# CAMMA-public/SelfPose3d

Hardware: AMD Instinct MI355X
Metric: multi-view samples/sec (5-view Panoptic, 80x80x20 voxel) (higher is better)
Workload: dtype f32

## Files before the change

include/sp3d.h:

```cpp
#ifndef SP3D_H
#define SP3D_H

#include <stdint.h>

#ifdef __cplusplus
extern "C" {
#endif

#define SP3D_ABI_VERSION 3
#define SP3D_MAX_VIEWS 16
#define SP3D_MAX_TOPK 32

#define SP3D_CAM_STRIDE 64
#define SP3D_CAM_R 0
#define SP3D_CAM_T 9
#define SP3D_CAM_F 12
#define SP3D_CAM_C 14
#define SP3D_CAM_K 16
#define SP3D_CAM_P 19
#define SP3D_CAM_A 21
#define SP3D_CAM_W0 27
#define SP3D_CAM_H0 28
#define SP3D_CAM_FLIP 29
#define SP3D_CAM_RXY 32
// ... 147 lines not shown
int sp3d_wino_fused_split(const float *x, const void *U3, float *y, const float *shift, const float *residual, int mode, int B,
                          int X, int Y, int Z, int C, int O, void *stream);

int sp3d_wino_fused_split64(const float *x, const void *U3, float *y, const float *shift, const float *residual, int mode,
                            int B, int X, int Y, int Z, int C, int O, void *stream);

int sp3d_conv3_split(const float *x, const void *W3, float *y, const float *shift, const float *residual, int mode, int B,
                     int X, int Y, int Z, int C, int O, void *stream);

int sp3d_upsample2x_scatter(const float *G, float *out, const float *shift, const float *skip, int64_t batch, int X, int Y,
                            int Z, int O, void *stream);

int sp3d_upsample2x_scatter_head(const float *G, float *head, const float *shift, const float *skip, const float *wout,
                                 const float *bout, int64_t batch, int X, int Y, int Z, int O, int J, void *stream);

#define SP3D_GBN_F32 0
#define SP3D_GBN_F64 1
#define SP3D_GBN_REPLICAS 16
#define SP3D_GBN_PLAIN 0
#define SP3D_GBN_RELU 1
#define SP3D_GBN_ADD_RELU 2
int64_t sp3d_gbn_workspace_bytes(int G, int C);
int sp3d_gbn_forward(const void *x, void *y, int dtype, const int32_t *group_of, const int32_t *group_samples, int N,
                     int64_t S, int C, int G, int G_update, const void *weight, const void *bias, void *running_mean,
                     void *running_var, double eps, double momentum, int mode, const void *residual, void *mean,
                     void *invstd, void *scale, void *shift, double *workspace, void *stream);
int sp3d_gbn_backward(const void *x, const void *dy, void *dx, int dtype, const int32_t *group_of,
                      const int32_t *group_samples, int N, int64_t S, int C, int G, const void *weight, const void *mean,
                      const void *invstd, const void *scale, const void *shift, int mode, const void *y,
                      void *grad_residual, void *grad_weight, void *grad_bias, void *k123, double *workspace, void *stream);
// ... 6 lines not shown
```

selfpose3d_amd/_lib.py:

```python
from __future__ import annotations

import ctypes as C
import os
from typing import Optional, Sequence

import torch

_HERE = os.path.dirname(os.path.abspath(__file__))
_DEFAULT_LIB_PATH = os.path.join(_HERE, "libsp3d.so")
NOPK_LIB_PATH = os.path.join(_HERE, "libsp3d_nopk.so")
LIB_PATH = os.environ.get("SP3D_LIB_PATH") or _DEFAULT_LIB_PATH

LAYOUT_PLANAR = 0
LAYOUT_NHWC = 1
OUT_CHANNELS_LAST = 0x100
HM_BF16 = 0x200
OUT_BF16 = 0x400
SCATTER_AUTO, SCATTER_PER_TAP, SCATTER_MERGE = 0, 2, 3
MAX_VIEWS = 16
MAX_TOPK = 32
ABI_VERSION = 3

EXPORTS = [
    "sp3d_abi_version", "sp3d_error_string", "sp3d_pack_heatmaps", "sp3d_unproject_fwd", "sp3d_unproject_bwd",
    "sp3d_nms_topk_workspace_bytes", "sp3d_nms_topk", "sp3d_nms_proposals", "sp3d_soft_argmax", "sp3d_unproject_fwd_indexed",
    "sp3d_unproject_bwd_indexed", "sp3d_unproject_fwd_strided", "sp3d_fetch_ring", "sp3d_maxpool2x_cl", "sp3d_crop_shift_act_cl", "sp3d_rfft3d", "sp3d_irfft3d", "sp3d_cfft2d", "sp3d_cfft2d_ex", "sp3d_zdft_fwd_cl", "sp3d_zdft_inv_cl", "sp3d_unproject_fwd_zdft", "sp3d_cfft2d_88_tiled", "sp3d_freq_contract_ty", "sp3d_soft_argmax_grid", "sp3d_soft_argmax_grid_train", "sp3d_soft_argmax_grid_bwd", "sp3d_channel_shift_act", "sp3d_pack_heatmaps_ex",
    "sp3d_unproject_fwd_train", "sp3d_unproject_bwd_packed", "sp3d_unproject_bwd_packed_det", "sp3d_fixed_to_float", "sp3d_gaussian_target_3d", "sp3d_render_root_heatmaps", "sp3d_freq_contract", "sp3d_freq_contract_ex", "sp3d_wino_input", "sp3d_wino_output", "sp3d_wino_fused", "sp3d_wino_fused_split", "sp3d_wino_fused_split64", "sp3d_conv3_split", "sp3d_camera_finish", "sp3d_upsample2x_scatter", "sp3d_upsample2x_scatter_head", "sp3d_render_joints_fwd", "sp3d_render_joints_bwd", "sp3d_gbn_workspace_bytes", "sp3d_gbn_forward", "sp3d_gbn_backward",
]

_lib = None


class Sp3dError(RuntimeError):
    pass


def shared_gpu() -> bool:
    v = os.environ.get("SP3D_SHARED_GPU")
    if v is not None:
        return v.lower() in ("1", "true", "yes", "on")
    if any(os.environ.get(k) not in (None, "") for k in ("HIP_VISIBLE_DEVICES", "CUDA_VISIBLE_DEVICES", "ROCR_VISIBLE_DEVICES",
                                                          "GPU_DEVICE_ORDINAL")):
# ... 749 lines not shown
    if not x.is_contiguous(memory_format=torch.channels_last_3d) or x.dtype != torch.float32:
        raise Sp3dError("upsample2x_head_: float32 channels_last_3d activations expected")
    O = int(w_gemm.shape[1]) // 8
    J = int(w_out.shape[0])
    G = torch.matmul(x.permute(0, 2, 3, 4, 1).reshape(-1, Cc), w_gemm)
    if tuple(skip.shape) != (B, O, 2 * X, 2 * Y, 2 * Z) or not skip.is_contiguous(memory_format=torch.channels_last_3d):
        skip = skip.contiguous(memory_format=torch.channels_last_3d)
    wo = w_out.reshape(J, O).contiguous().float()
    bo = (b_out if b_out is not None else torch.zeros(J, device=x.device)).contiguous().float()
    head = torch.empty((B, 2 * X, 2 * Y, 2 * Z, J), dtype=torch.float32, device=x.device)
    check(lib.sp3d_upsample2x_scatter_head(G.data_ptr(), head.data_ptr(), shift.data_ptr(), skip.data_ptr(), wo.data_ptr(),
                                           bo.data_ptr(), B, X, Y, Z, O, J, _stream(x.device)), "sp3d_upsample2x_scatter_head")
    return head.permute(0, 4, 1, 2, 3)


class _RenderJoints(torch.autograd.Function):
    @staticmethod
    def forward(ctx, kps, count, h, w, sigma):
        lib = load()
        _require_cuda(kps, "kps")
        N, Pn, J = (int(v) for v in kps.shape[:3])
        k = kps.contiguous().float()
        cnt = None if count is None else count.to(device=kps.device, dtype=torch.int32).contiguous()
        out = torch.empty((N, J, h, w), dtype=torch.float32, device=kps.device)
        check(lib.sp3d_render_joints_fwd(k.data_ptr(), cnt.data_ptr() if cnt is not None else None, N, Pn, J, h, w,
                                         float(sigma), out.data_ptr(), _stream(kps.device)), "sp3d_render_joints_fwd")
        ctx.save_for_backward(k, cnt if cnt is not None else torch.empty(0, device=kps.device))
        ctx.geom = (h, w, float(sigma), cnt is not None, kps.dtype)
        return out if kps.dtype == torch.float32 else out.to(kps.dtype)

# ... 16 lines not shown
```

selfpose3d_amd/build.py:

```python
from __future__ import annotations

import os
import subprocess
import sys

HERE = os.path.dirname(os.path.abspath(__file__))
CSRC = os.path.join(HERE, "csrc")
SOURCES = ["sp3d_unproject.hip", "sp3d_proposal.hip", "sp3d_epilogue.hip", "sp3d_synth.hip", "sp3d_fftconv.hip", "sp3d_winograd.hip", "sp3d_fft.hip", "sp3d_gbn.hip"]
HEADERS = [os.path.join("..", "pk_src1.py"), "sp3d_device.h", "sp3d_proj_pk.h", "sp3d_tuning.h", "sp3d_twiddles.h", os.path.join("..", "..", "include", "sp3d.h")]
LIB = os.path.join(HERE, "libsp3d.so")
HIPCC = os.environ.get("HIPCC", "/opt/rocm/bin/hipcc")
FLAGS = ["--offload-arch=gfx950", "-O3", "-std=c++17", "-ffp-contract=off", "-munsafe-fp-atomics", "-fPIC", "-shared",
         "-Wall", "-Wno-unused-function"]
LINK = ["-L/opt/rocm/lib", "-lhipfft"]


def needs_build() -> bool:
    if not os.path.exists(LIB):
        return True
    t = os.path.getmtime(LIB)
    deps = [os.path.join(CSRC, s) for s in SOURCES + HEADERS] + [os.path.abspath(__file__)]
    return any(os.path.getmtime(d) > t for d in deps if os.path.exists(d))


PER_SOURCE_FLAGS = {"sp3d_winograd.hip": ["-fno-slp-vectorize"],
                    "sp3d_fft.hip": ["-fno-slp-vectorize"], "sp3d_fftconv.hip": ["-fno-slp-vectorize"]}


LLVM_BIN = os.environ.get("SP3D_LLVM_BIN", "/opt/rocm/lib/llvm/bin")

NOPK_LIB = os.path.join(HERE, "libsp3d_nopk.so")
NOPK_FLAGS = ["-DSP3D_NO_PK", "-fno-slp-vectorize", "-Xclang", "-target-feature", "-Xclang", "-packed-fp32-ops"]




def _compile_one(src: str, objdir: str, cflags, verbose: bool, host_flags=()) -> str:
    from . import pk_src1
    base = os.path.join(objdir, src.replace(".hip", ""))
    path = os.path.join(CSRC, src)
    cuid = "-cuid=" + src.replace(".", "_")
# ... 85 lines not shown
```

selfpose3d_amd/csrc/sp3d_winograd.hip:

```cpp
#include <hip/hip_runtime.h>
#include <stdint.h>

#include "../../include/sp3d.h"

namespace sp3d {

__device__ __forceinline__ void bt4(float &d0, float &d1, float &d2, float &d3)
{
    const float t0 = d0 - d2, t1 = d1 + d2, t2 = d2 - d1, t3 = d1 - d3;
    d0 = t0; d1 = t1; d2 = t2; d3 = t3;
}

__global__ __launch_bounds__(256) void wino_input_kernel(const float *__restrict__ x, float *__restrict__ V, int B, int X,
                                                        int Y, int Z, int C, int TX, int TY, int TZ)
{
    const int64_t T = (int64_t)B * TX * TY * TZ;
    const int64_t gid = (int64_t)blockIdx.x * 256 + threadIdx.x;
    if (gid >= T * C) return;
    const int c = (int)(gid % C);
    int64_t t = gid / C;
    const int tz = (int)(t % TZ); int64_t r = t / TZ;
    const int ty = (int)(r % TY); r /= TY;
    const int tx = (int)(r % TX);
    const int b = (int)(r / TX);
// ... 858 lines not shown

__device__ __forceinline__ void split3(const float4 a, u32x4 &q0, u32x4 &q1)
{
    const unsigned hi01 = pack_bf16(a.x, a.y), hi23 = pack_bf16(a.z, a.w);
    const float r0 = __builtin_amdgcn_fmed3f(a.x - bf16_lo(hi01), 0.0f, a.x - bf16_lo(hi01));
    const float r1 = __builtin_amdgcn_fmed3f(a.y - bf16_hi(hi01), 0.0f, a.y - bf16_hi(hi01));
    const float r2 = __builtin_amdgcn_fmed3f(a.z - bf16_lo(hi23), 0.0f, a.z - bf16_lo(hi23));
    const float r3 = __builtin_amdgcn_fmed3f(a.w - bf16_hi(hi23), 0.0f, a.w - bf16_hi(hi23));
    const unsigned mid01 = pack_bf16(r0, r1), mid23 = pack_bf16(r2, r3);
    const unsigned lo01 = pack_bf16(r0 - bf16_lo(mid01), r1 - bf16_hi(mid01));
    const unsigned lo23 = pack_bf16(r2 - bf16_lo(mid23), r3 - bf16_hi(mid23));
    q0 = u32x4{lo01, lo23, hi01, hi23};
    q1 = u32x4{hi01, hi23, mid01, mid23};
}

template <int C, int MODE>
__global__ __launch_bounds__(64 * (4 + CD_PROD)) __attribute__((amdgpu_waves_per_eu(2, 2)))
void conv3_split_kernel(const float *__restrict__ x, const unsigned *__restrict__ W3, float *__restrict__ y,
                        const float *__restrict__ shift, const float *__restrict__ res, int B, int X, int Y, int Z, int NBX,
                        int NBY, int NBZ, int nblocks)
{
    constexpr int O = 32, NCH = C / 8;
    extern __shared__ __attribute__((aligned(16))) unsigned cd_lds[];
    const int tid = threadIdx.x, lane = tid & 63, wave = tid >> 6, t = lane & 31, h = lane >> 5;
    const int my_blocks = ((int)blockIdx.x < nblocks) ? (nblocks - 1 - (int)blockIdx.x) / (int)gridDim.x + 1 : 0;
    const int n_items = my_blocks * NCH;
    auto decode = [&](int item, int &b, int &ox0, int &oy0, int &oz0) {
        int bid = (int)blockIdx.x + (item / NCH) * (int)gridDim.x;
        const int bz = bid % NBZ; bid /= NBZ;
        const int by = bid % NBY; bid /= NBY;
        const int bx = bid % NBX;
        b = bid / NBX;
        ox0 = bx * CD_BX; oy0 = by * CD_BY; oz0 = bz * CD_BZ;
    };

// ... 121 lines not shown
            }
#pragma unroll
            for (int r = 0; r < 9; ++r) {
                __builtin_amdgcn_sched_group_barrier(0x008, 1, 0);
                __builtin_amdgcn_sched_group_barrier(0x020, 1, 0);
            }
            __builtin_amdgcn_sched_group_barrier(0x008, 15, 0);
            __builtin_amdgcn_sched_barrier(0);
            a0 = a1;
            w0 = w1;
        }
        CD_STAMP(1);
        if (cc == NCH - 1) {
            int b, ox0, oy0, oz0;
            decode(item, b, ox0, oy0, oz0);
            if (ox0 + CD_BX <= X && oy0 + CD_BY <= Y && oz0 + CD_BZ <= Z) {
                const float sh = shift[t];
                const int64_t obase = ((((int64_t)b * X + ox0 + 4 * wave) * Y + oy0 + 4 * h) * Z + oz0) * O + t;
#pragma unroll
                for (int i = 0; i < 4; ++i)
#pragma unroll
                    for (int v = 0; v < 16; ++v) {
                        const int64_t idx = obase + (((int64_t)i * Y + (v & 3)) * Z + (v >> 2)) * O;
                        float val = acc[i][v] + sh;
                        if (MODE == 2) val += res[idx];
                        if (MODE >= 1) val = fmaxf(val, 0.0f);
                        if (MODE == 3) val += res[idx];
#if SP3D_W16_ABLATE & 16
                        if (val == 123.456f)
#endif
                        y[idx] = val;
// ... 9 lines not shown
                __builtin_amdgcn_fence(__ATOMIC_RELEASE, "wavefront");
                __builtin_amdgcn_wave_barrier();
#pragma unroll
                for (int r = 0; r < 4; ++r) {
                    const int m = (lane >> 3) + 8 * r;
                    float4 a = *reinterpret_cast<const float4 *>(scr + m * 32 + 4 * g);
                    const int xo = ox0 + 4 * wave + mb, yo = oy0 + (m & 7), zo = oz0 + (m >> 3);
                    if (xo < X && yo < Y && zo < Z) {
                        const int64_t vox = (((int64_t)b * X + xo) * Y + yo) * Z + zo;
                        a.x += sh4.x; a.y += sh4.y; a.z += sh4.z; a.w += sh4.w;
                        float4 rr = make_float4(0.0f, 0.0f, 0.0f, 0.0f);
                        if (MODE >= 2) rr = *reinterpret_cast<const float4 *>(res + vox * O + 4 * g);
                        if (MODE == 2) { a.x += rr.x; a.y += rr.y; a.z += rr.z; a.w += rr.w; }
                        if (MODE >= 1) { a.x = fmaxf(a.x, 0.0f); a.y = fmaxf(a.y, 0.0f); a.z = fmaxf(a.z, 0.0f); a.w = fmaxf(a.w, 0.0f); }
                        if (MODE == 3) { a.x += rr.x; a.y += rr.y; a.z += rr.z; a.w += rr.w; }
#if SP3D_W16_ABLATE & 16
                        if (a.x == 123.456f)
#endif
                        *reinterpret_cast<float4 *>(y + vox * O + 4 * g) = a;
                    }
                }
                __builtin_amdgcn_fence(__ATOMIC_RELEASE, "wavefront");
                __builtin_amdgcn_wave_barrier();
            }
            }
        }
        CD_STAMP(2);
        __syncthreads();
        CD_STAMP(3);
    }
}


}
// ... 63 lines not shown
    const int64_t blocks = (int64_t)B * NBX * NBY * NBZ;
    if (blocks > 0x7fffffff) return SP3D_ERANGE;
    constexpr int nbw = 2, ks = 2;
    hipStream_t s = (hipStream_t)stream;
    const unsigned *u3 = reinterpret_cast<const unsigned *>(U3);
    const dim3 grid((unsigned)blocks), block(64 * (4 / nbw) * ks);
#define SP3D_WF(C_, M_) hipLaunchKernelGGL((wino_fused16_kernel<C_, M_, 2, 2>), grid, block, 0, s, x, u3, y, shift, residual, B, X, Y, Z, NBX, NBY, NBZ)
#define SP3D_WFM(C_) switch (mode) { case 0: SP3D_WF(C_, 0); break; case 1: SP3D_WF(C_, 1); break; case 2: SP3D_WF(C_, 2); break; default: SP3D_WF(C_, 3); }
    if (C == 32) { SP3D_WFM(32) } else { SP3D_WFM(64) }
#undef SP3D_WFM
#undef SP3D_WF
    const hipError_t e = hipGetLastError();
    return e == hipSuccess ? SP3D_OK : (int)e;
}

extern "C" int sp3d_conv3_split(const float *x, const void *W3, float *y, const float *shift, const float *residual, int mode,
                                int B, int X, int Y, int Z, int C, int O, void *stream)
{
    using namespace sp3d;
    if (B <= 0 || X <= 0 || Y <= 0 || Z <= 0 || mode < 0 || mode > 3) return SP3D_EINVAL;
    if (!x || !W3 || !y || !shift || (mode >= 2 && !residual)) return SP3D_ENULL;
    if (O != 32 || (C != 16 && C != 32) || (reinterpret_cast<uintptr_t>(W3) & 15)) return SP3D_EUNSUPPORTED;
    if (reinterpret_cast<uintptr_t>(y) & 15) return SP3D_EUNSUPPORTED;
    if ((int64_t)X * Y * Z * C * 2 > 0x7fffffff) return SP3D_ERANGE;
    const int NBX = (X + CD_BX - 1) / CD_BX, NBY = (Y + CD_BY - 1) / CD_BY, NBZ = (Z + CD_BZ - 1) / CD_BZ;
    const int64_t blocks = (int64_t)B * NBX * NBY * NBZ;
    if (blocks > 0x7fffffff) return SP3D_ERANGE;
    static int cu_count[64] = {0};
    int dev = 0, cus = 256;
    if (hipGetDevice(&dev) == hipSuccess && dev >= 0 && dev < 64) {
        if (cu_count[dev] == 0) {
            int n = 0;
            cu_count[dev] = (hipDeviceGetAttribute(&n, hipDeviceAttributeMultiprocessorCount, dev) == hipSuccess && n > 0) ? n : 256;
        }
        cus = cu_count[dev];
    }
    const int rounds = (int)((blocks + cus - 1) / cus);
    const int nwg = (int)((blocks + rounds - 1) / rounds);
    const dim3 grid((unsigned)nwg), block(64 * (4 + CD_PROD));
    const size_t lds = (size_t)2 * CD_BUFS * sizeof(unsigned) + 4 * 1024 * sizeof(float);
    hipStream_t s = (hipStream_t)stream;
    const unsigned *w3 = reinterpret_cast<const unsigned *>(W3);
    int cd_dev = 0;
    { const hipError_t ed = hipGetDevice(&cd_dev); if (ed != hipSuccess) return (int)ed; }
    if (cd_dev < 0 || cd_dev >= 64) cd_dev = 63;
#define SP3D_CD(C_, M_) { static bool attr_dev[64] = {}; bool &attr = attr_dev[cd_dev]; if (!attr || cd_dev == 63) { hipError_t ea = hipFuncSetAttribute(reinterpret_cast<const void *>(conv3_split_kernel<C_, M_>), hipFuncAttributeMaxDynamicSharedMemorySize, (int)lds); if (ea != hipSuccess) return (int)ea; attr = true; } \
    hipLaunchKernelGGL((conv3_split_kernel<C_, M_>), grid, block, lds, s, x, w3, y, shift, residual, B, X, Y, Z, NBX, NBY, NBZ, (int)blocks); }
#define SP3D_CDI(C_) switch (mode) { case 0: SP3D_CD(C_, 0); break; case 1: SP3D_CD(C_, 1); break; case 2: SP3D_CD(C_, 2); break; default: SP3D_CD(C_, 3); }
    if (C == 16) { SP3D_CDI(16) } else { SP3D_CDI(32) }
#undef SP3D_CDI
#undef SP3D_CD
    const hipError_t e = hipGetLastError();
    return e == hipSuccess ? SP3D_OK : (int)e;
}

extern "C" int sp3d_debug_conv3_timeline(void *dev_buffer)
{
#ifdef SP3D_CD_TIMELINE
    unsigned long long *p = (unsigned long long *)dev_buffer;
    return (int)hipMemcpyToSymbol(HIP_SYMBOL(sp3d::g_cd_tl), &p, sizeof(p));
#else
    (void)dev_buffer;
    return SP3D_EUNSUPPORTED;
#endif
}
```

selfpose3d_amd/v2v_net.py:

```python
from __future__ import annotations

import torch
import torch.nn as nn
import torch.nn.functional as F


def _bn(c):
    from .grouped_bn import GroupedBatchNorm3d
    return GroupedBatchNorm3d(c)


def _grouped(bn, training: bool) -> bool:
    return training and getattr(bn, "groups", None) is not None


def fft_len(n: int) -> int:
    m = n + (n & 1)
    while True:
        r, odd = m, 0
        for q in (2, 3, 5, 7, 11, 13):
            if q > 2 and r % q == 0:
                odd += 1
            while r % q == 0:
                r //= q
# ... 185 lines not shown
                    u._sp3d_direct = _lib.conv_weights_split(wc)
            for u in (u1, u2):
                if u is not None and u.shape[2] == 32 and u.shape[1] in (16, 32):
                    u._sp3d_split = _lib.wino_weights_split(u)
                elif u is not None and u.shape[2] == 64 and u.shape[1] in (32, 64):
                    u._sp3d_split = _lib.wino_weights_split(u, 16)
            if len(blk.skip_con) > 0:
                ws, ss = self._fold(blk.skip_con[0], blk.skip_con[1])
                t[name] = (w1, s1, w2, (s2 + ss).contiguous(), ws, u1, u2)
            else:
                t[name] = (w1, s1, w2, s2, None, u1, u2)
        res("front_res", n.front_layers[1])
        ed = n.encoder_decoder
        for name in ("encoder_res1", "encoder_res2", "mid_res", "decoder_res2", "decoder_res1", "skip_res1", "skip_res2"):
            res(name, getattr(ed, name))
        for name in ("decoder_upsample2", "decoder_upsample1"):
            blk = getattr(ed, name).block
            wT, sT = self._fold(blk[0], blk[1], transposed=True)
            wg = wT.permute(0, 2, 3, 4, 1).reshape(wT.shape[0], 8 * wT.shape[1]).contiguous()
            t[name] = (wT, sT, wg)
        self.t = t

    def _conv3(self, x, w, u, shift, mode, residual=None):
        from . import _lib
        if u is not None and self.net.winograd and x.is_contiguous(memory_format=torch.channels_last_3d) \
                and not x.is_contiguous():
            B, C, X, Y, Z = x.shape
            T = B * ((X + 1) // 2) * ((Y + 1) // 2) * ((Z + 1) // 2)
            u3 = getattr(u, "_sp3d_split", None) if getattr(self.net, "wino_split", True) else None
            if u3 is not None and u.shape[2] == 64:
                return _lib.wino_fused_conv3d_(x, u, shift, mode, residual, u3)
            if C >= 128 or (C >= 64 and 64 * T * C * 4 <= 160e6):
                return _lib.wino_conv3d_(x, u, shift, mode, residual)
            w3 = getattr(u, "_sp3d_direct", None) if getattr(self.net, "wino_split", True) and getattr(self.net, "direct_conv", True) else None
# ... 203 lines not shown
        else:
            buf = self._fft_buffer(B, cin, S, x.device)
            buf[:, :, :X, :Y, :Z].copy_(x[:, :cin])
        Yf = _lib.freq_contract(_lib.rfft3d(buf), self.t[wkey])
        y = _lib.irfft3d_(Yf, S[2])
        w1 = self.t["front_res"][0]
        cl = w1.is_contiguous(memory_format=torch.channels_last_3d) and not w1.is_contiguous()
        if cl and y.is_contiguous() and y.shape[1] % 4 == 0 and Z % 4 == 0 and 4 * Z * (y.shape[1] + 4) * 4 <= 65536:
            return _lib.crop_shift_act_cl(y, X, Y, Z, s0, True)
        y = y[:, :, :X, :Y, :Z]
        y = y.contiguous(memory_format=torch.channels_last_3d if cl else torch.contiguous_format)
        return _lib.channel_shift_act_(y, s0, 1)

    def _tail(self, x):
        from . import _lib
        x = self._res(x, "front_res")
        skip1 = self._res(x, "skip_res1")
        x = self._res(self._pool(x), "encoder_res1")
        skip2 = self._res(x, "skip_res2")
        x = self._res(self._pool(x), "encoder_res2")
        x = self._res(self._res(x, "mid_res"), "decoder_res2")
        x = self._up2x(x, "decoder_upsample2", skip2)
        x = self._res(x, "decoder_res1")
        o = self.net.output_layer
        wT, sT, wg = self.t["decoder_upsample1"]
        if self.net.winograd and self._is_cl(x) and wg.is_cuda and wT.shape[1] == 32 and x.dtype == torch.float32:
            return _lib.upsample2x_head_(x, wg, sT, skip1, o.weight, o.bias)
        x = self._up2x(x, "decoder_upsample1", skip1)
        return self._conv1(x, o.weight, o.bias)

    def _pool(self, x):
        from . import _lib
        if self._is_cl(x) and x.is_cuda and x.dtype == torch.float32 and x.shape[1] % 4 == 0 and \
                all(int(v) % 2 == 0 for v in x.shape[2:]):
            return _lib.maxpool2x(x)
        return F.max_pool3d(x, 2, 2)

    @staticmethod
    def _is_cl(x):
        return x.is_contiguous(memory_format=torch.channels_last_3d) and not x.is_contiguous()

    def _up2x(self, x, name, skip):
        from . import _lib
        wT, sT, wg = self.t[name]
        if self.net.winograd and self._is_cl(x) and wg.is_cuda and wT.shape[1] % 4 == 0:
            return _lib.upsample2x_(x, wg, sT, skip)
        return _lib.channel_shift_act_(F.conv_transpose3d(x, wT, None, 2), sT, 3, skip)

    def _conv1(self, x, w, bias=None):
        if self.net.winograd and self._is_cl(x) and x.is_cuda:
            B, C, X, Y, Z = x.shape
            O = w.shape[0]
            x2 = x.permute(0, 2, 3, 4, 1).reshape(-1, C)
            y = torch.matmul(x2, w.reshape(O, C).t()) if bias is None else torch.addmm(bias, x2, w.reshape(O, C).t())
            return y.view(B, X, Y, Z, O).permute(0, 4, 1, 2, 3)
        return F.conv3d(x, w, bias, 1, 0)


class V2VNet(nn.Module):
    def __init__(self, input_channels: int, output_channels: int):
        super().__init__()
        self.front_layers = nn.Sequential(ConvBnRelu3d(input_channels, 16, 7), Residual3d(16, 32))
# ... 97 lines not shown
```

Measured before the change: 2746.

## Fuse transposed-conv upsample GEMM with scatter and output head via split-bf16 MFMA

Adds a new kernel that does the 2x transposed-conv upsample as an in-kernel GEMM on bf16 MFMA units. It splits operands into hi/mid/lo bf16 pieces to keep near-f32 accuracy, and fuses the shift, skip add and scatter into the same kernel. This replaces the torch.matmul intermediate G plus a separate scatter kernel. A head variant also folds the final 1x1 output conv into the epilogue. An optional path fuses the J-channel head into the skip_res1 conv3 kernel, off by default. The aim is to cut the intermediate tensor's memory traffic and launches, at the cost of extra MFMA work for the precision split and heavy LDS use.

```diff
diff --git a/include/sp3d.h b/include/sp3d.h
--- a/include/sp3d.h
+++ b/include/sp3d.h
@@ -185,6 +185,16 @@
 int sp3d_upsample2x_scatter_head(const float *G, float *head, const float *shift, const float *skip, const float *wout,
                                  const float *bout, int64_t batch, int X, int Y, int Z, int O, int J, void *stream);
 
+int sp3d_upsample2x_gemm(const float *x, const void *W3, float *out, const float *shift, const float *skip, int B, int X,
+                         int Y, int Z, int C, int O, void *stream);
+
+int sp3d_upsample2x_gemm_head(const float *x, const void *W3, float *head, const float *shift, const float *skip,
+                              const float *wout, const float *bout, int B, int X, int Y, int Z, int C, int O, int J,
+                              int skip_j, void *stream);
+
+int sp3d_conv3_split_head(const float *x, const void *W3, float *head, const float *shift, const float *residual,
+                          const float *wout, int B, int X, int Y, int Z, int C, int O, int J, void *stream);
+
 #define SP3D_GBN_F32 0
 #define SP3D_GBN_F64 1
 #define SP3D_GBN_REPLICAS 16
diff --git a/selfpose3d_amd/_lib.py b/selfpose3d_amd/_lib.py
--- a/selfpose3d_amd/_lib.py
+++ b/selfpose3d_amd/_lib.py
@@ -25,7 +25,7 @@
     "sp3d_abi_version", "sp3d_error_string", "sp3d_pack_heatmaps", "sp3d_unproject_fwd", "sp3d_unproject_bwd",
     "sp3d_nms_topk_workspace_bytes", "sp3d_nms_topk", "sp3d_nms_proposals", "sp3d_soft_argmax", "sp3d_unproject_fwd_indexed",
     "sp3d_unproject_bwd_indexed", "sp3d_unproject_fwd_strided", "sp3d_fetch_ring", "sp3d_maxpool2x_cl", "sp3d_crop_shift_act_cl", "sp3d_rfft3d", "sp3d_irfft3d", "sp3d_cfft2d", "sp3d_cfft2d_ex", "sp3d_zdft_fwd_cl", "sp3d_zdft_inv_cl", "sp3d_unproject_fwd_zdft", "sp3d_cfft2d_88_tiled", "sp3d_freq_contract_ty", "sp3d_soft_argmax_grid", "sp3d_soft_argmax_grid_train", "sp3d_soft_argmax_grid_bwd", "sp3d_channel_shift_act", "sp3d_pack_heatmaps_ex",
-    "sp3d_unproject_fwd_train", "sp3d_unproject_bwd_packed", "sp3d_unproject_bwd_packed_det", "sp3d_fixed_to_float", "sp3d_gaussian_target_3d", "sp3d_render_root_heatmaps", "sp3d_freq_contract", "sp3d_freq_contract_ex", "sp3d_wino_input", "sp3d_wino_output", "sp3d_wino_fused", "sp3d_wino_fused_split", "sp3d_wino_fused_split64", "sp3d_conv3_split", "sp3d_camera_finish", "sp3d_upsample2x_scatter", "sp3d_upsample2x_scatter_head", "sp3d_render_joints_fwd", "sp3d_render_joints_bwd", "sp3d_gbn_workspace_bytes", "sp3d_gbn_forward", "sp3d_gbn_backward",
+    "sp3d_unproject_fwd_train", "sp3d_unproject_bwd_packed", "sp3d_unproject_bwd_packed_det", "sp3d_fixed_to_float", "sp3d_gaussian_target_3d", "sp3d_render_root_heatmaps", "sp3d_freq_contract", "sp3d_freq_contract_ex", "sp3d_wino_input", "sp3d_wino_output", "sp3d_wino_fused", "sp3d_wino_fused_split", "sp3d_wino_fused_split64", "sp3d_conv3_split", "sp3d_camera_finish", "sp3d_upsample2x_scatter", "sp3d_upsample2x_scatter_head", "sp3d_upsample2x_gemm", "sp3d_upsample2x_gemm_head", "sp3d_conv3_split_head", "sp3d_render_joints_fwd", "sp3d_render_joints_bwd", "sp3d_gbn_workspace_bytes", "sp3d_gbn_forward", "sp3d_gbn_backward",
 ]
 
 _lib = None
@@ -805,6 +805,97 @@
     return head.permute(0, 4, 1, 2, 3)
 
 
+def upsample_weights_split(w_gemm: torch.Tensor) -> torch.Tensor:
+    Cc, N = (int(v) for v in w_gemm.shape)
+    w = w_gemm.float()
+    hi = w.bfloat16()
+    r = w - hi.float()
+    mid = r.bfloat16()
+    lo = (r - mid.float()).bfloat16()
+    pieces = torch.stack([lo, hi, mid, hi], 0).reshape(4, Cc // 8, 2, 4, N)
+    return pieces.permute(1, 2, 4, 0, 3).contiguous()
+
+
+def _upsample_args(x: torch.Tensor, W3: torch.Tensor, shift: torch.Tensor, skip: torch.Tensor, skip_c: Optional[int],
+                   what: str):
+    _require_cuda(x, "x")
+    B, Cc, X, Y, Z = (int(v) for v in x.shape)
+    if not x.is_contiguous(memory_format=torch.channels_last_3d) or x.dtype != torch.float32:
+        raise Sp3dError(f"{what}: float32 channels_last_3d activations expected")
+    if W3.dtype != torch.bfloat16 or not W3.is_contiguous() or tuple(W3.shape[:2]) != (Cc // 8, 2) or W3.shape[2] % 8:
+        raise Sp3dError(f"{what}: weight records of upsample_weights_split expected")
+    O = int(W3.shape[2]) // 8
+    if shift.dtype != torch.float32 or not shift.is_contiguous() or shift.numel() != O or shift.device != x.device:
+        raise Sp3dError(f"{what}: shift must be {O} contiguous float32 values on the activations' device")
+    want = (B, O if skip_c is None else skip_c, 2 * X, 2 * Y, 2 * Z)
+    if skip.dtype != torch.float32 or tuple(skip.shape) != want or skip.device != x.device:
+        raise Sp3dError(f"{what}: float32 skip of shape {want} expected")
+    if not skip.is_contiguous(memory_format=torch.channels_last_3d):
+        skip = skip.contiguous(memory_format=torch.channels_last_3d)
+    return B, Cc, X, Y, Z, O, skip
+
+
+def upsample2x_gemm_(x: torch.Tensor, W3: torch.Tensor, shift: torch.Tensor, skip: torch.Tensor) -> torch.Tensor:
+    lib = load()
+    B, Cc, X, Y, Z, O, skip = _upsample_args(x, W3, shift, skip, None, "upsample2x_gemm_")
+    out = torch.empty((B, 2 * X, 2 * Y, 2 * Z, O), dtype=torch.float32, device=x.device).permute(0, 4, 1, 2, 3)
+    lib.sp3d_upsample2x_gemm.restype = C.c_int
+    lib.sp3d_upsample2x_gemm.argtypes = [C.c_void_p] * 5 + [C.c_int] * 6 + [C.c_void_p]
+    check(lib.sp3d_upsample2x_gemm(x.data_ptr(), W3.data_ptr(), out.data_ptr(), shift.data_ptr(), skip.data_ptr(), B, X, Y,
+                                   Z, Cc, O, _stream(x.device)), "sp3d_upsample2x_gemm")
+    return out
+
+
+def _head_weights(w_out: torch.Tensor, b_out: Optional[torch.Tensor], O: int, device):
+    J = int(w_out.shape[0])
+    if w_out.numel() != J * O:
+        raise Sp3dError(f"head weights: (J, {O}, 1, 1, 1) expected, got {tuple(w_out.shape)}")
+    wo = w_out.reshape(J, O).contiguous().float()
+    bo = (b_out if b_out is not None else torch.zeros(J, device=device)).contiguous().float()
+    if bo.numel() != J:
+        raise Sp3dError(f"head bias: {J} values expected")
+    return J, wo, bo
+
+
+def upsample2x_gemm_head_(x: torch.Tensor, W3: torch.Tensor, shift: torch.Tensor, skip: torch.Tensor, w_out: torch.Tensor,
+                          b_out: torch.Tensor, skip_head: bool = False) -> torch.Tensor:
+    lib = load()
+    J = int(w_out.shape[0])
+    B, Cc, X, Y, Z, O, skip = _upsample_args(x, W3, shift, skip, J if skip_head else None, "upsample2x_gemm_head_")
+    J, wo, bo = _head_weights(w_out, b_out, O, x.device)
+    head = torch.empty((B, 2 * X, 2 * Y, 2 * Z, J), dtype=torch.float32, device=x.device)
+    lib.sp3d_upsample2x_gemm_head.restype = C.c_int
+    lib.sp3d_upsample2x_gemm_head.argtypes = [C.c_void_p] * 7 + [C.c_int] * 8 + [C.c_void_p]
+    check(lib.sp3d_upsample2x_gemm_head(x.data_ptr(), W3.data_ptr(), head.data_ptr(), shift.data_ptr(), skip.data_ptr(),
+                                        wo.data_ptr(), bo.data_ptr(), B, X, Y, Z, Cc, O, J, int(bool(skip_head)),
+                                        _stream(x.device)), "sp3d_upsample2x_gemm_head")
+    return head.permute(0, 4, 1, 2, 3)
+
+
+def conv3_split_head_(x: torch.Tensor, W3: torch.Tensor, shift: torch.Tensor, residual: torch.Tensor,
+                      w_out: torch.Tensor) -> torch.Tensor:
+    lib = load()
+    _require_cuda(x, "x")
+    B, Cc, X, Y, Z = (int(v) for v in x.shape)
+    if not x.is_contiguous(memory_format=torch.channels_last_3d) or x.dtype != torch.float32:
+        raise Sp3dError("conv3_split_head_: float32 channels_last_3d activations expected")
+    O = int(W3.shape[3])
+    J = int(w_out.shape[0])
+    if w_out.numel() != J * O:
+        raise Sp3dError(f"head weights: (J, {O}, 1, 1, 1) expected, got {tuple(w_out.shape)}")
+    wo = w_out.reshape(J, O).contiguous().float()
+    if tuple(residual.shape) != (B, O, X, Y, Z) or residual.dtype != torch.float32:
+        raise Sp3dError("conv3_split_head_: float32 residual of the result's shape expected")
+    if not residual.is_contiguous(memory_format=torch.channels_last_3d):
+        residual = residual.contiguous(memory_format=torch.channels_last_3d)
+    head = torch.empty((B, X, Y, Z, J), dtype=torch.float32, device=x.device)
+    lib.sp3d_conv3_split_head.restype = C.c_int
+    lib.sp3d_conv3_split_head.argtypes = [C.c_void_p] * 6 + [C.c_int] * 7 + [C.c_void_p]
+    check(lib.sp3d_conv3_split_head(x.data_ptr(), W3.data_ptr(), head.data_ptr(), shift.data_ptr(), residual.data_ptr(),
+                                    wo.data_ptr(), B, X, Y, Z, Cc, O, J, _stream(x.device)), "sp3d_conv3_split_head")
+    return head.permute(0, 4, 1, 2, 3)
+
+
 class _RenderJoints(torch.autograd.Function):
     @staticmethod
     def forward(ctx, kps, count, h, w, sigma):
diff --git a/selfpose3d_amd/build.py b/selfpose3d_amd/build.py
--- a/selfpose3d_amd/build.py
+++ b/selfpose3d_amd/build.py
@@ -6,7 +6,7 @@
 
 HERE = os.path.dirname(os.path.abspath(__file__))
 CSRC = os.path.join(HERE, "csrc")
-SOURCES = ["sp3d_unproject.hip", "sp3d_proposal.hip", "sp3d_epilogue.hip", "sp3d_synth.hip", "sp3d_fftconv.hip", "sp3d_winograd.hip", "sp3d_fft.hip", "sp3d_gbn.hip"]
+SOURCES = ["sp3d_unproject.hip", "sp3d_proposal.hip", "sp3d_epilogue.hip", "sp3d_synth.hip", "sp3d_fftconv.hip", "sp3d_winograd.hip", "sp3d_fft.hip", "sp3d_gbn.hip", "sp3d_upconv.hip"]
 HEADERS = [os.path.join("..", "pk_src1.py"), "sp3d_device.h", "sp3d_proj_pk.h", "sp3d_tuning.h", "sp3d_twiddles.h", os.path.join("..", "..", "include", "sp3d.h")]
 LIB = os.path.join(HERE, "libsp3d.so")
 HIPCC = os.environ.get("HIPCC", "/opt/rocm/bin/hipcc")
@@ -24,7 +24,8 @@
 
 
 PER_SOURCE_FLAGS = {"sp3d_winograd.hip": ["-fno-slp-vectorize"],
-                    "sp3d_fft.hip": ["-fno-slp-vectorize"], "sp3d_fftconv.hip": ["-fno-slp-vectorize"]}
+                    "sp3d_fft.hip": ["-fno-slp-vectorize"], "sp3d_fftconv.hip": ["-fno-slp-vectorize"],
+                    "sp3d_upconv.hip": ["-fno-slp-vectorize"]}
 
 
 LLVM_BIN = os.environ.get("SP3D_LLVM_BIN", "/opt/rocm/lib/llvm/bin")
diff --git a/selfpose3d_amd/csrc/sp3d_upconv.hip b/selfpose3d_amd/csrc/sp3d_upconv.hip
--- /dev/null
+++ b/selfpose3d_amd/csrc/sp3d_upconv.hip
@@ -0,0 +1,261 @@
+#include <hip/hip_runtime.h>
+#include <stdint.h>
+
+#include "../../include/sp3d.h"
+
+namespace sp3d {
+
+typedef float f32x16_u __attribute__((ext_vector_type(16)));
+typedef unsigned u32x4_u __attribute__((ext_vector_type(4)));
+typedef __bf16 bf16x8_u __attribute__((ext_vector_type(8)));
+typedef __bf16 bf16x2_u __attribute__((ext_vector_type(2)));
+typedef float f32x2_u __attribute__((ext_vector_type(2)));
+
+constexpr int UP_WAVES = 8, UP_LDS_BYTES = 131072, UP_MAX_J = 64;
+constexpr __host__ __device__ int up_vb(int C) { return C <= 64 ? 2 : 1; }
+
+static __device__ __forceinline__ unsigned up_pack_bf16(float a, float b)
+{
+    f32x2_u f = {a, b};
+    return __builtin_bit_cast(unsigned, __builtin_convertvector(f, bf16x2_u));
+}
+static __device__ __forceinline__ float up_bf16_lo(unsigned u) { return __uint_as_float(u << 16); }
+static __device__ __forceinline__ float up_bf16_hi(unsigned u) { return __uint_as_float(u & 0xffff0000u); }
+
+static __device__ __forceinline__ f32x16_u up_mfma(u32x4_u a, u32x4_u b, f32x16_u c)
+{
+    return __builtin_amdgcn_mfma_f32_32x32x16_bf16(__builtin_bit_cast(bf16x8_u, a), __builtin_bit_cast(bf16x8_u, b), c, 0, 0, 0);
+}
+
+static __device__ __forceinline__ void up_split(const float4 a, u32x4_u &x0, u32x4_u &x1, u32x4_u &x2)
+{
+    const unsigned hi01 = up_pack_bf16(a.x, a.y), hi23 = up_pack_bf16(a.z, a.w);
+    const float r0 = __builtin_amdgcn_fmed3f(a.x - up_bf16_lo(hi01), 0.0f, a.x - up_bf16_lo(hi01));
+    const float r1 = __builtin_amdgcn_fmed3f(a.y - up_bf16_hi(hi01), 0.0f, a.y - up_bf16_hi(hi01));
+    const float r2 = __builtin_amdgcn_fmed3f(a.z - up_bf16_lo(hi23), 0.0f, a.z - up_bf16_lo(hi23));
+    const float r3 = __builtin_amdgcn_fmed3f(a.w - up_bf16_hi(hi23), 0.0f, a.w - up_bf16_hi(hi23));
+    const unsigned mid01 = up_pack_bf16(r0, r1), mid23 = up_pack_bf16(r2, r3);
+    const unsigned lo01 = up_pack_bf16(r0 - up_bf16_lo(mid01), r1 - up_bf16_hi(mid01));
+    const unsigned lo23 = up_pack_bf16(r2 - up_bf16_lo(mid23), r3 - up_bf16_hi(mid23));
+    x0 = u32x4_u{hi01, hi23, lo01, lo23};
+    x1 = u32x4_u{hi01, hi23, hi01, hi23};
+    x2 = u32x4_u{mid01, mid23, mid01, mid23};
+}
+
+template <int C, int O, bool HEAD, bool SKIPJ = false>
+__global__ __launch_bounds__(64 * UP_WAVES) void upsample2x_gemm_kernel(
+    const float *__restrict__ x, const unsigned *__restrict__ W3, float *__restrict__ out, const float *__restrict__ shift,
+    const float *__restrict__ skip, const float *__restrict__ wout, const float *__restrict__ bout, int64_t n_in, int X,
+    int Y, int Z, int J)
+{
+    constexpr int NCH = C / 8, NCOL = 8 * O, SLAB = UP_LDS_BYTES / (C * 8);
+    constexpr int PLANE = NCH * 2 * SLAB;
+    static_assert(SLAB % 64 == 0 && UP_WAVES % (SLAB / 64) == 0 && NCOL % SLAB == 0 && O % 32 == 0, "column slab");
+    static_assert(!HEAD || (O == 32 && SLAB == NCOL), "head form: all 256 columns of O = 32 in one workgroup");
+    static_assert(HEAD || !SKIPJ, "a J-channel skip belongs to the head form");
+    constexpr int CG = SLAB / 64;
+    constexpr int VB = up_vb(C);
+    constexpr int VG = UP_WAVES / CG;
+    constexpr int TILE = 32 * VB * VG;
+    extern __shared__ __attribute__((aligned(16))) u32x4_u up_lds[];
+    const u32x4_u *__restrict__ W = reinterpret_cast<const u32x4_u *>(W3);
+    float *hw = reinterpret_cast<float *>(up_lds + 2 * PLANE);
+
+    const int tid = threadIdx.x, lane = tid & 63, wave = tid >> 6, t = lane & 31, h = lane >> 5;
+    const int cg = wave % CG, vg = wave / CG;
+    const int slab = blockIdx.y;
+    const int64_t ntiles = (n_in + TILE - 1) / TILE;
+
+    float4 d[NCH][VB];
+    auto load_x = [&](int64_t tile) {
+        const int64_t n0 = tile * TILE + 32 * VB * vg + t;
+#pragma unroll
+        for (int vb = 0; vb < VB; ++vb) {
+            const int64_t n = n0 + 32 * vb;
+            const float *p = x + (n < n_in ? n : n_in - 1) * C + 4 * h;
+#pragma unroll
+            for (int k = 0; k < NCH; ++k) d[k][vb] = *reinterpret_cast<const float4 *>(p + 8 * k);
+        }
+    };
+    int64_t tile = blockIdx.x;
+    if (tile < ntiles) load_x(tile);
+
+    constexpr int NST = 2 * PLANE / (64 * UP_WAVES), BATCH = 8;
+    static_assert(NST % BATCH == 0, "");
+#pragma unroll
+    for (int i0 = 0; i0 < NST; i0 += BATCH) {
+        u32x4_u tmp[BATCH];
+#pragma unroll
+        for (int u = 0; u < BATCH; ++u) {
+            const int i = tid + (i0 + u) * 64 * UP_WAVES, q = i & 1, r = i >> 1, col = r % SLAB, kh = r / SLAB;
+            tmp[u] = W[((int64_t)kh * NCOL + slab * SLAB + col) * 2 + q];
+        }
+#pragma unroll
+        for (int u = 0; u < BATCH; ++u) {
+            const int i = tid + (i0 + u) * 64 * UP_WAVES;
+            up_lds[(i & 1) * PLANE + (i >> 1)] = tmp[u];
+        }
+    }
+    if (HEAD) {
+        for (int i = tid; i < J * 32; i += 64 * UP_WAVES) hw[i] = wout[i];
+        for (int i = tid; i < J; i += 64 * UP_WAVES) hw[J * 32 + i] = bout[i];
+    }
+    __syncthreads();
+
+    for (; tile < ntiles; tile += gridDim.x) {
+        f32x16_u acc[2][VB];
+#pragma unroll
+        for (int cb = 0; cb < 2; ++cb)
+#pragma unroll
+            for (int vb = 0; vb < VB; ++vb)
+#pragma unroll
+                for (int v = 0; v < 16; ++v) acc[cb][vb][v] = 0.0f;
+#pragma unroll
+        for (int k = 0; k < NCH; ++k) {
+            u32x4_u xa[VB][3];
+#pragma unroll
+            for (int vb = 0; vb < VB; ++vb) up_split(d[k][vb], xa[vb][0], xa[vb][1], xa[vb][2]);
+#pragma unroll
+            for (int cb = 0; cb < 2; ++cb) {
+                const int r = (k * 2 + h) * SLAB + 64 * cg + 32 * cb + t;
+                const u32x4_u w0 = up_lds[r], w2 = up_lds[PLANE + r];
+                const u32x4_u w1 = __builtin_shufflevector(w0, w2, 2, 3, 4, 5);
+#pragma unroll
+                for (int vb = 0; vb < VB; ++vb) {
+                    acc[cb][vb] = up_mfma(w0, xa[vb][0], acc[cb][vb]);
+                    acc[cb][vb] = up_mfma(w1, xa[vb][1], acc[cb][vb]);
+                    acc[cb][vb] = up_mfma(w2, xa[vb][2], acc[cb][vb]);
+                }
+            }
+            __builtin_amdgcn_sched_barrier(0);
+        }
+        const int64_t cur = tile;
+        if (tile + gridDim.x < ntiles) load_x(tile + gridDim.x);
+
+        int64_t child[VB][2];
+        float4 k4[VB][2][4];
+#pragma unroll
+        for (int vb = 0; vb < VB; ++vb) {
+            const unsigned n = (unsigned)min(cur * TILE + 32 * VB * vg + 32 * vb + t, n_in - 1);
+            const unsigned z = n % (unsigned)Z, m = n / (unsigned)Z, y = m % (unsigned)Y, m2 = m / (unsigned)Y;
+            const unsigned xx = m2 % (unsigned)X, b = m2 / (unsigned)X;
+#pragma unroll
+            for (int cb = 0; cb < 2; ++cb) {
+                const int col0 = slab * SLAB + 64 * cg + 32 * cb;
+                const int ijk = col0 / O, o0 = col0 % O;
+                child[vb][cb] = (((int64_t)b * (2 * X) + 2 * xx + (ijk >> 2)) * (2 * Y) + 2 * y + ((ijk >> 1) & 1)) * (2 * Z) +
+                                2 * z + (ijk & 1);
+#pragma unroll
+                for (int g = 0; g < 4; ++g)
+                    k4[vb][cb][g] = SKIPJ ? make_float4(0.0f, 0.0f, 0.0f, 0.0f)
+                                          : *reinterpret_cast<const float4 *>(skip + child[vb][cb] * O + o0 + 8 * g + 4 * h);
+            }
+        }
+#pragma unroll
+        for (int vb = 0; vb < VB; ++vb) {
+            if (cur * TILE + 32 * VB * vg + 32 * vb + t >= n_in) continue;
+#pragma unroll
+            for (int cb = 0; cb < 2; ++cb) {
+                const int o0 = (slab * SLAB + 64 * cg + 32 * cb) % O;
+                const int64_t ch = child[vb][cb];
+                float4 v[4];
+#pragma unroll
+                for (int g = 0; g < 4; ++g) {
+                    const int o = o0 + 8 * g + 4 * h;
+                    const float4 s = *reinterpret_cast<const float4 *>(shift + o);
+                    v[g].x = fmaxf(acc[cb][vb][4 * g + 0] + s.x, 0.0f) + k4[vb][cb][g].x;
+                    v[g].y = fmaxf(acc[cb][vb][4 * g + 1] + s.y, 0.0f) + k4[vb][cb][g].y;
+                    v[g].z = fmaxf(acc[cb][vb][4 * g + 2] + s.z, 0.0f) + k4[vb][cb][g].z;
+                    v[g].w = fmaxf(acc[cb][vb][4 * g + 3] + s.w, 0.0f) + k4[vb][cb][g].w;
+                    if (!HEAD) *reinterpret_cast<float4 *>(out + ch * O + o) = v[g];
+                }
+                if (HEAD) {
+                    for (int j = 0; j < J; ++j) {
+                        const float *wj = hw + j * 32 + 4 * h;
+                        float p = 0.0f;
+#pragma unroll
+                        for (int g = 0; g < 4; ++g) {
+                            const float4 w = *reinterpret_cast<const float4 *>(wj + 8 * g);
+                            p = fmaf(v[g].x, w.x, p); p = fmaf(v[g].y, w.y, p);
+                            p = fmaf(v[g].z, w.z, p); p = fmaf(v[g].w, w.w, p);
+                        }
+                        p += __shfl_xor(p, 32);
+                        if ((j & 1) == h) out[ch * J + j] = SKIPJ ? (p + skip[ch * J + j]) + hw[J * 32 + j] : p + hw[J * 32 + j];
+                    }
+                }
+            }
+        }
+    }
+}
+
+}
+
+namespace {
+
+template <int C, int O, bool HEAD, bool SKIPJ = false>
+int up_launch(const float *x, const void *W, float *out, const float *shift, const float *skip, const float *wout,
+              const float *bout, int B, int X, int Y, int Z, int J, void *stream)
+{
+    using namespace sp3d;
+    constexpr int SLAB = UP_LDS_BYTES / (C * 8), TILE = 32 * up_vb(C) * (UP_WAVES / (SLAB / 64));
+    const int64_t n_in = (int64_t)B * X * Y * Z;
+    const int64_t ntiles = (n_in + TILE - 1) / TILE;
+    const int slabs = 8 * O / SLAB;
+    static int cu_count[64] = {0};
+    int dev = 0, cus = 256;
+    hipError_t e = hipGetDevice(&dev);
+    if (e != hipSuccess) return (int)e;
+    if (dev >= 0 && dev < 64) {
+        if (cu_count[dev] == 0) {
+            int n = 0;
+            cu_count[dev] = (hipDeviceGetAttribute(&n, hipDeviceAttributeMultiprocessorCount, dev) == hipSuccess && n > 0) ? n : 256;
+        }
+        cus = cu_count[dev];
+    }
+    const int64_t per = cus / slabs > 0 ? cus / slabs : 1;
+    const int64_t gx = ntiles < per ? ntiles : per;
+    const size_t lds = (size_t)UP_LDS_BYTES + (HEAD ? (size_t)J * 33 * sizeof(float) : 0);
+    auto kern = upsample2x_gemm_kernel<C, O, HEAD, SKIPJ>;
+    static bool attr_dev[64] = {};
+    if (dev < 0 || dev >= 64 || !attr_dev[dev]) {
+        e = hipFuncSetAttribute(reinterpret_cast<const void *>(kern), hipFuncAttributeMaxDynamicSharedMemorySize,
+                                UP_LDS_BYTES + (HEAD ? UP_MAX_J * 33 * (int)sizeof(float) : 0));
+        if (e != hipSuccess) return (int)e;
+        if (dev >= 0 && dev < 64) attr_dev[dev] = true;
+    }
+    hipLaunchKernelGGL(kern, dim3((unsigned)gx, (unsigned)slabs), dim3(64 * UP_WAVES), lds, (hipStream_t)stream, x,
+                       reinterpret_cast<const unsigned *>(W), out, shift, skip, wout, bout, n_in, X, Y, Z, J);
+    e = hipGetLastError();
+    return e == hipSuccess ? SP3D_OK : (int)e;
+}
+
+}
+
+extern "C" int sp3d_upsample2x_gemm(const float *x, const void *W3, float *out, const float *shift, const float *skip, int B,
+                                    int X, int Y, int Z, int C, int O, void *stream)
+{
+    if (B <= 0 || X <= 0 || Y <= 0 || Z <= 0 || C <= 0 || O <= 0) return SP3D_EINVAL;
+    if (!x || !W3 || !out || !shift || !skip) return SP3D_ENULL;
+    if ((reinterpret_cast<uintptr_t>(x) | reinterpret_cast<uintptr_t>(W3) | reinterpret_cast<uintptr_t>(out) |
+         reinterpret_cast<uintptr_t>(shift) | reinterpret_cast<uintptr_t>(skip)) & 15) return SP3D_EUNSUPPORTED;
+    if ((int64_t)B * X * Y * Z >= ((int64_t)1 << 31)) return SP3D_ERANGE;
+    if (C == 64 && O == 32) return up_launch<64, 32, false>(x, W3, out, shift, skip, nullptr, nullptr, B, X, Y, Z, 0, stream);
+    if (C == 128 && O == 64) return up_launch<128, 64, false>(x, W3, out, shift, skip, nullptr, nullptr, B, X, Y, Z, 0, stream);
+    return SP3D_EUNSUPPORTED;
+}
+
+extern "C" int sp3d_upsample2x_gemm_head(const float *x, const void *W3, float *head, const float *shift, const float *skip,
+                                         const float *wout, const float *bout, int B, int X, int Y, int Z, int C, int O,
+                                         int J, int skip_j, void *stream)
+{
+    if (B <= 0 || X <= 0 || Y <= 0 || Z <= 0 || C <= 0 || O <= 0 || J <= 0) return SP3D_EINVAL;
+    if (!x || !W3 || !head || !shift || !skip || !wout || !bout) return SP3D_ENULL;
+    if ((reinterpret_cast<uintptr_t>(x) | reinterpret_cast<uintptr_t>(W3) | reinterpret_cast<uintptr_t>(shift) |
+         reinterpret_cast<uintptr_t>(skip)) & 15) return SP3D_EUNSUPPORTED;
+    if (J > sp3d::UP_MAX_J) return SP3D_EUNSUPPORTED;
+    if ((int64_t)B * X * Y * Z >= ((int64_t)1 << 31)) return SP3D_ERANGE;
+    if (C == 64 && O == 32 && skip_j)
+        return up_launch<64, 32, true, true>(x, W3, head, shift, skip, wout, bout, B, X, Y, Z, J, stream);
+    if (C == 64 && O == 32) return up_launch<64, 32, true>(x, W3, head, shift, skip, wout, bout, B, X, Y, Z, J, stream);
+    return SP3D_EUNSUPPORTED;
+}
diff --git a/selfpose3d_amd/csrc/sp3d_winograd.hip b/selfpose3d_amd/csrc/sp3d_winograd.hip
--- a/selfpose3d_amd/csrc/sp3d_winograd.hip
+++ b/selfpose3d_amd/csrc/sp3d_winograd.hip
@@ -896,11 +896,11 @@
     q1 = u32x4{hi01, hi23, mid01, mid23};
 }
 
-template <int C, int MODE>
+template <int C, int MODE, bool HEAD = false>
 __global__ __launch_bounds__(64 * (4 + CD_PROD)) __attribute__((amdgpu_waves_per_eu(2, 2)))
 void conv3_split_kernel(const float *__restrict__ x, const unsigned *__restrict__ W3, float *__restrict__ y,
                         const float *__restrict__ shift, const float *__restrict__ res, int B, int X, int Y, int Z, int NBX,
-                        int NBY, int NBZ, int nblocks)
+                        int NBY, int NBZ, int nblocks, const float *__restrict__ wout, int J)
 {
     constexpr int O = 32, NCH = C / 8;
     extern __shared__ __attribute__((aligned(16))) unsigned cd_lds[];
@@ -1052,7 +1052,7 @@
         if (cc == NCH - 1) {
             int b, ox0, oy0, oz0;
             decode(item, b, ox0, oy0, oz0);
-            if (ox0 + CD_BX <= X && oy0 + CD_BY <= Y && oz0 + CD_BZ <= Z) {
+            if (!HEAD && ox0 + CD_BX <= X && oy0 + CD_BY <= Y && oz0 + CD_BZ <= Z) {
                 const float sh = shift[t];
                 const int64_t obase = ((((int64_t)b * X + ox0 + 4 * wave) * Y + oy0 + 4 * h) * Z + oz0) * O + t;
 #pragma unroll
@@ -1092,10 +1092,25 @@
                         if (MODE == 2) { a.x += rr.x; a.y += rr.y; a.z += rr.z; a.w += rr.w; }
                         if (MODE >= 1) { a.x = fmaxf(a.x, 0.0f); a.y = fmaxf(a.y, 0.0f); a.z = fmaxf(a.z, 0.0f); a.w = fmaxf(a.w, 0.0f); }
                         if (MODE == 3) { a.x += rr.x; a.y += rr.y; a.z += rr.z; a.w += rr.w; }
+                        if (HEAD) {
+                            for (int j0 = 0; j0 < J; j0 += 8) {
+                                float mine = 0.0f;
+                                for (int jj = 0; jj < 8 && j0 + jj < J; ++jj) {
+                                    const float4 w = *reinterpret_cast<const float4 *>(wout + (j0 + jj) * 32 + 4 * g);
+                                    float p = fmaf(a.w, w.w, fmaf(a.z, w.z, fmaf(a.y, w.y, a.x * w.x)));
+                                    p += __shfl_xor(p, 1);
+                                    p += __shfl_xor(p, 2);
+                                    p += __shfl_xor(p, 4);
+                                    if (jj == g) mine = p;
+                                }
+                                if (j0 + g < J) y[vox * J + j0 + g] = mine;
+                            }
+                        } else {
 #if SP3D_W16_ABLATE & 16
                         if (a.x == 123.456f)
 #endif
                         *reinterpret_cast<float4 *>(y + vox * O + 4 * g) = a;
+                        }
                     }
                 }
                 __builtin_amdgcn_fence(__ATOMIC_RELEASE, "wavefront");
@@ -1189,8 +1204,8 @@
     return e == hipSuccess ? SP3D_OK : (int)e;
 }
 
-extern "C" int sp3d_conv3_split(const float *x, const void *W3, float *y, const float *shift, const float *residual, int mode,
-                                int B, int X, int Y, int Z, int C, int O, void *stream)
+static int conv3_split_launch(const float *x, const void *W3, float *y, const float *shift, const float *residual, int mode,
+                              int B, int X, int Y, int Z, int C, int O, const float *wout, int J, void *stream)
 {
     using namespace sp3d;
     if (B <= 0 || X <= 0 || Y <= 0 || Z <= 0 || mode < 0 || mode > 3) return SP3D_EINVAL;
@@ -1219,14 +1234,31 @@
     int cd_dev = 0;
     { const hipError_t ed = hipGetDevice(&cd_dev); if (ed != hipSuccess) return (int)ed; }
     if (cd_dev < 0 || cd_dev >= 64) cd_dev = 63;
-#define SP3D_CD(C_, M_) { static bool attr_dev[64] = {}; bool &attr = attr_dev[cd_dev]; if (!attr || cd_dev == 63) { hipError_t ea = hipFuncSetAttribute(reinterpret_cast<const void *>(conv3_split_kernel<C_, M_>), hipFuncAttributeMaxDynamicSharedMemorySize, (int)lds); if (ea != hipSuccess) return (int)ea; attr = true; } \
-    hipLaunchKernelGGL((conv3_split_kernel<C_, M_>), grid, block, lds, s, x, w3, y, shift, residual, B, X, Y, Z, NBX, NBY, NBZ, (int)blocks); }
-#define SP3D_CDI(C_) switch (mode) { case 0: SP3D_CD(C_, 0); break; case 1: SP3D_CD(C_, 1); break; case 2: SP3D_CD(C_, 2); break; default: SP3D_CD(C_, 3); }
-    if (C == 16) { SP3D_CDI(16) } else { SP3D_CDI(32) }
+#define SP3D_CD(C_, M_, H_) { static bool attr_dev[64] = {}; bool &attr = attr_dev[cd_dev]; if (!attr || cd_dev == 63) { hipError_t ea = hipFuncSetAttribute(reinterpret_cast<const void *>(conv3_split_kernel<C_, M_, H_>), hipFuncAttributeMaxDynamicSharedMemorySize, (int)lds); if (ea != hipSuccess) return (int)ea; attr = true; } \
+    hipLaunchKernelGGL((conv3_split_kernel<C_, M_, H_>), grid, block, lds, s, x, w3, y, shift, residual, B, X, Y, Z, NBX, NBY, NBZ, (int)blocks, wout, J); }
+#define SP3D_CDI(C_) switch (mode) { case 0: SP3D_CD(C_, 0, false); break; case 1: SP3D_CD(C_, 1, false); break; case 2: SP3D_CD(C_, 2, false); break; default: SP3D_CD(C_, 3, false); }
+    if (wout) {
+        if (C == 16) SP3D_CD(16, 2, true) else SP3D_CD(32, 2, true)
+    } else if (C == 16) { SP3D_CDI(16) } else { SP3D_CDI(32) }
 #undef SP3D_CDI
 #undef SP3D_CD
     const hipError_t e = hipGetLastError();
     return e == hipSuccess ? SP3D_OK : (int)e;
+}
+
+extern "C" int sp3d_conv3_split(const float *x, const void *W3, float *y, const float *shift, const float *residual, int mode,
+                                int B, int X, int Y, int Z, int C, int O, void *stream)
+{
+    return conv3_split_launch(x, W3, y, shift, residual, mode, B, X, Y, Z, C, O, nullptr, 0, stream);
+}
+
+extern "C" int sp3d_conv3_split_head(const float *x, const void *W3, float *head, const float *shift, const float *residual,
+                                     const float *wout, int B, int X, int Y, int Z, int C, int O, int J, void *stream)
+{
+    if (B <= 0 || X <= 0 || Y <= 0 || Z <= 0 || J <= 0) return SP3D_EINVAL;
+    if (!x || !W3 || !head || !shift || !residual || !wout) return SP3D_ENULL;
+    if (J > 64 || (reinterpret_cast<uintptr_t>(wout) & 15)) return SP3D_EUNSUPPORTED;
+    return conv3_split_launch(x, W3, head, shift, residual, 2, B, X, Y, Z, C, O, wout, J, stream);
 }
 
 extern "C" int sp3d_debug_conv3_timeline(void *dev_buffer)
diff --git a/selfpose3d_amd/v2v_net.py b/selfpose3d_amd/v2v_net.py
--- a/selfpose3d_amd/v2v_net.py
+++ b/selfpose3d_amd/v2v_net.py
@@ -223,10 +223,13 @@
         ed = n.encoder_decoder
         for name in ("encoder_res1", "encoder_res2", "mid_res", "decoder_res2", "decoder_res1", "skip_res1", "skip_res2"):
             res(name, getattr(ed, name))
+        from . import _lib
         for name in ("decoder_upsample2", "decoder_upsample1"):
             blk = getattr(ed, name).block
             wT, sT = self._fold(blk[0], blk[1], transposed=True)
             wg = wT.permute(0, 2, 3, 4, 1).reshape(wT.shape[0], 8 * wT.shape[1]).contiguous()
+            if wg.is_cuda and (int(wT.shape[0]), int(wT.shape[1])) in ((64, 32), (128, 64)):
+                wg._sp3d_split = _lib.upsample_weights_split(wg)
             t[name] = (wT, sT, wg)
         self.t = t
 
@@ -460,20 +463,43 @@
 
     def _tail(self, x):
         from . import _lib
+        o = self.net.output_layer
+        wT, sT, wg = self.t["decoder_upsample1"]
         x = self._res(x, "front_res")
-        skip1 = self._res(x, "skip_res1")
+        head = self.net.winograd and self._is_cl(x) and wg.is_cuda and wT.shape[1] == 32 and x.dtype == torch.float32
+        w3 = self._upconv_split(wg) if head and int(o.weight.shape[0]) <= 64 else None
+        skip_head = self._res_head(x, "skip_res1", o.weight) \
+            if w3 is not None and getattr(self.net, "fused_skip_head", False) else None
+        skip1 = skip_head if skip_head is not None else self._res(x, "skip_res1")
         x = self._res(self._pool(x), "encoder_res1")
         skip2 = self._res(x, "skip_res2")
         x = self._res(self._pool(x), "encoder_res2")
         x = self._res(self._res(x, "mid_res"), "decoder_res2")
         x = self._up2x(x, "decoder_upsample2", skip2)
         x = self._res(x, "decoder_res1")
-        o = self.net.output_layer
-        wT, sT, wg = self.t["decoder_upsample1"]
-        if self.net.winograd and self._is_cl(x) and wg.is_cuda and wT.shape[1] == 32 and x.dtype == torch.float32:
+        if skip_head is not None or (head and self._is_cl(x)):
+            if not self._is_cl(x):
+                raise RuntimeError("V2V plan: the decoder left channels-last after the J-channel skip was formed")
+            if w3 is not None:
+                return _lib.upsample2x_gemm_head_(x, w3, sT, skip1, o.weight, o.bias, skip_head=skip_head is not None)
             return _lib.upsample2x_head_(x, wg, sT, skip1, o.weight, o.bias)
         x = self._up2x(x, "decoder_upsample1", skip1)
         return self._conv1(x, o.weight, o.bias)
+
+    def _res_head(self, x, name, w_out):
+        from . import _lib
+        w1, s1, w2, s2, ws, u1, u2 = self.t[name]
+        net = self.net
+        if ws is not None or u2 is None or not self._is_cl(x) or x.dtype != torch.float32 or \
+                not (getattr(net, "wino_split", True) and getattr(net, "direct_conv", True)):
+            return None
+        w3 = getattr(u2, "_sp3d_direct", None)
+        if w3 is None or int(w2.shape[1]) not in (16, 32) or int(u2.shape[2]) != 32:
+            return None
+        h = self._conv3(x, w1, u1, s1, 1)
+        if not self._is_cl(h):
+            return None
+        return _lib.conv3_split_head_(h, w3, s2, x, w_out)
 
     def _pool(self, x):
         from . import _lib
@@ -490,8 +516,17 @@
         from . import _lib
         wT, sT, wg = self.t[name]
         if self.net.winograd and self._is_cl(x) and wg.is_cuda and wT.shape[1] % 4 == 0:
+            w3 = self._upconv_split(wg)
+            if w3 is not None and x.dtype == torch.float32:
+                return _lib.upsample2x_gemm_(x, w3, sT, skip)
             return _lib.upsample2x_(x, wg, sT, skip)
         return _lib.channel_shift_act_(F.conv_transpose3d(x, wT, None, 2), sT, 3, skip)
+
+    def _upconv_split(self, wg):
+        import os
+        if not getattr(self.net, "fused_tail", os.environ.get("SP3D_FUSED_TAIL", "1") not in ("0", "")):
+            return None
+        return getattr(wg, "_sp3d_split", None)
 
     def _conv1(self, x, w, bias=None):
         if self.net.winograd and self._is_cl(x) and x.is_cuda:
```

Result: faster. 2800, median of 6 (+2.0%).
